# SketchyScene/SketchySceneColorization

Hardware: AMD Instinct MI355X
Metric: train images/sec (192x192, gen+disc fwd+bwd) (higher is better)
Workload: dtype fp32 (bf16x6 split on the bf16 MFMA, fp32 accumulate; filter gradients and few-channel layers on the exact-fp32 MFMA); 1 GPU; Foreground_Instance_Colorization Pix2Pix GAN train step (D-step + G-step, TF-Adam), 192x192, batch 32 per GPU; global_batch=32, parallelism=dp1, ranks_observed_by_allreduce=1, launcher=in-process, block_type=Pix2Pix, launch=hipGraph replay

## Files before the change

include/sketchycolor_hip.h:

```cpp
#ifndef SKETCHYCOLOR_HIP_H
#define SKETCHYCOLOR_HIP_H

#include <stdint.h>

#ifdef __cplusplus
extern "C" {
#endif

#define SSC_ACT_NONE 0
#define SSC_ACT_RELU 1
#define SSC_ACT_LRELU 2
#define SSC_ACT_TANH 3
#define SSC_ACT_PRELU 5
#define SSC_ACT_MIU 4

typedef struct ssc_gview {
    const float* s0;
    const float* s1;
    const float* ab0;
    const float* ab1;
    int32_t C0, C1;
    int32_t H, W;
    int32_t act;
    int32_t act1;
// ... 38 lines not shown
    int32_t ws_kc;
    const void* wsplit;
    int32_t ws_nbp;
    int32_t lds_hint;
} ssc_conv_desc;
#define SSC_SK_FLAG_WORDS 8192
typedef struct ssc_split_job {
    const float* w;
    void* dst;
    int32_t taps, c0, c1, orient;
    int64_t first_thread;
} ssc_split_job;
int ssc_filter_split_geom(int taps, int c0, int c1, int orient, int* kc, int* nbp, int64_t* bytes, int64_t* threads);
int ssc_filter_split(const float* w, int taps, int c0, int c1, int orient, void* dst, void* stream);
int ssc_bf16_prepare(void);
int ssc_filter_split_batch(const ssc_split_job* jobs_dev, int njobs, int64_t total_threads, void* stream);

int ssc_sk_configure(int timeout_ms, int test_withhold);

typedef struct ssc_wgrad_desc {
    ssc_gview g;
    ssc_gview d;
    float* out;
    int32_t NB, PH, PW;
    int32_t TH, TW, in_stride, ioff_y, ioff_x;
    int32_t Cg_real;
    int32_t Nn;
    int32_t ldc;
    int32_t accumulate;
    int32_t exact;
    int32_t _pad;
} ssc_wgrad_desc;

int ssc_version(void);
int ssc_build_hash(char* buf, int len);
int ssc_device_info(int* cu_count, int* wave_size, char* arch, int arch_len);

int ssc_conv_forward(const ssc_conv_desc* d, float* ws, int64_t ws_bytes, void* stream);
int ssc_conv_wgrad(const ssc_wgrad_desc* d, float* ws, int64_t ws_bytes, void* stream);
int ssc_conv_wgrad128_supported(const ssc_wgrad_desc* d);
int ssc_conv_wgrad128(const ssc_wgrad_desc* d, float* ws, int64_t ws_bytes, void* stream);
int ssc_conv_wgn16_supported(const ssc_wgrad_desc* d);
int ssc_conv_forward_bn(const ssc_conv_desc* d, float* ws, int64_t ws_bytes, const float* scale, const float* offset,
                        float eps, float* ab, float* stats, void* stream);
int ssc_head1_forward_supported(const ssc_conv_desc* d);
int ssc_head1_forward(const ssc_conv_desc* d, float* ws, int64_t ws_bytes, void* stream);
int ssc_head1_dgrad_supported(const ssc_conv_desc* d);
int ssc_head1_dgrad(const ssc_conv_desc* d, void* stream);
int ssc_head1_wgrad_supported(const ssc_wgrad_desc* d);
int ssc_head1_wgrad(const ssc_wgrad_desc* d, float* ws, int64_t ws_bytes, void* stream);
int ssc_head1_dgrad_bn_backward(const ssc_conv_desc* d, const float* x, const float* ab, const float* stats, int act,
                                const float* rowb, float rowb_scale, float* dx, float* dscale, float* doffset, float* ws,
                                int64_t ws_bytes, void* stream);
int ssc_bn_bwd_finalize(const float* partial, int nblk, int C, int64_t M, float* coef, float* dscale, float* doffset,
                        void* stream);
int ssc_conv_narrow_supported(const ssc_conv_desc* d);
int ssc_conv_narrow_forward(const ssc_conv_desc* d, void* stream);
int ssc_conv_pw1x1_supported(const ssc_conv_desc* d);
int ssc_conv_c3x3_supported(const ssc_conv_desc* d);
int ssc_conv_s2n16_supported(const ssc_conv_desc* d);
int ssc_conv_tr4n16_supported(const ssc_conv_desc* d);
int ssc_conv_fewchan7_supported(const ssc_conv_desc* d);
int ssc_conv_tr4_tiny_supported(const ssc_conv_desc* d);
int ssc_conv_fewchan_supported(const ssc_conv_desc* d);
int ssc_conv_forward_kernel_name(const ssc_conv_desc* d, char* buf, int len);
int ssc_conv_wgrad_kernel_name(const ssc_wgrad_desc* d, char* buf, int len);
int ssc_conv_forward_plan(const ssc_conv_desc* d, int64_t ws_bytes, int* out5);
#define SSC_RIDER_BN 0
#define SSC_RIDER_BNBWD 1
#define SSC_RIDER_BNBWD2 2
#define SSC_RIDER_MINMAX 3
#define SSC_RIDER_PATH_PLAIN 0
#define SSC_RIDER_PATH_STREAM 1
#define SSC_RIDER_PATH_TILE 2
#define SSC_RIDER_PATH_SLAB 3
#define SSC_RIDER_ROWS_NONE 0
#define SSC_RIDER_ROWS_WS_HEAD 1
#define SSC_RIDER_ROWS_WS_TAIL 2
#define SSC_RIDER_ROWS_CALLER 3
struct ssc_bnbwd_site;
int ssc_conv_rider_plan(const ssc_conv_desc* d, int rider, int64_t ws_bytes, const struct ssc_bnbwd_site* site0,
                        const struct ssc_bnbwd_site* site1, int C0, int64_t* out5);
int ssc_conv_wgrad_plan(const ssc_wgrad_desc* d, int64_t ws_bytes, int* out4);
int ssc_conv_wgrad128_plan(const ssc_wgrad_desc* d, int64_t ws_bytes, int* out7);
int ssc_conv_bf_plan(const ssc_conv_desc* d, int64_t ws_bytes, int* out10);
int ssc_conv_stream_plan(const ssc_conv_desc* d, int* out4);

int ssc_nchw_to_nhwc(const float* src, float* dst, int N, int C, int HW, int ldc, int coff, void* stream);
int ssc_nhwc_to_nchw(const float* src, float* dst, int N, int C, int HW, int ldc, int coff, void* stream);
int ssc_sketch_preprocess_u8(const uint8_t* src, int N, int H, int W, int thicken, float* dst, void* stream);
int ssc_image_postprocess_u8(const float* src, int ldc, int coff, int64_t M, uint8_t* dst, void* stream);
int ssc_bg_stage_u8(const uint8_t* fg, const uint8_t* bg, const int32_t* labels, int64_t M, float* inputs, float* targets,
                    float* xd_real, float* count, void* workspace, int64_t workspace_bytes, void* stream);
int ssc_bg_stage_cached_u8(const uint8_t* fg_cache, int64_t S_fg, const uint8_t* bg_cache, int64_t S_bg, const uint8_t* seg_cache,
                           int64_t S_seg, const int32_t* slot, const uint8_t* recolor, int64_t N, int64_t P, float* inputs,
                           float* targets, float* xd_real, int32_t* labels, float* count, void* workspace,
                           int64_t workspace_bytes, void* stream);
int ssc_bg_finish_u8(const float* img, int ldc, const uint8_t* fg, const uint8_t* mask, int64_t M, uint8_t* out,
                     void* stream);
int ssc_image_metrics_u8(const uint8_t* a, const uint8_t* b, const uint8_t* mask, int N, int H, int W, const double* win11,
                         double* out, void* ws, int64_t ws_bytes, void* stream);
int ssc_image_metrics_f32(const float* a, int lda, int coff_a, const float* b, int ldb, int coff_b, int b_planar, int N, int H,
                          int W, const double* win11, double* out, void* ws, int64_t ws_bytes, void* stream);
int ssc_image_metrics_bg_f32(const float* img, int ldc, const uint8_t* fg, const uint8_t* target, const uint8_t* mask, int N, int H,
                             int W, const double* win11, double* out, void* ws, int64_t ws_bytes, void* stream);
int ssc_color_metrics_u8(const uint8_t* a, const uint8_t* b, const uint8_t* mask, int N, int H, int W, const double* lin256,
// ... 244 lines not shown
```

sketchyscenecolorization_amd/build.py:

```python
import os
import subprocess
import sys

HERE = os.path.dirname(os.path.abspath(__file__))
ROOT = os.path.dirname(HERE)
CSRC = os.path.join(HERE, 'csrc')
LIB_DIR = os.path.join(HERE, 'lib')
LIB_PATH = os.path.join(LIB_DIR, 'libsketchycolor_hip.so')
EXTRA_FLAGS = {'igemm.hip': ['-Xclang', '-target-feature', '-Xclang', '-load-store-opt']} if os.environ.get('SSC_NO_LSOPT') == '1' else {}
NO_PACKED_FP32 = {'narrow.hip': []}
VGPR_FORM = ['-mllvm', '-amdgpu-mfma-vgpr-form=1']
LAST_BUILD = None
SOURCES = ['igemm.hip', 'igemm_bf16.hip', 'wgrad128.hip', 'wgrad128_bf16.hip', 'wgn16.hip', 'narrow.hip', 'head1.hip', 'fewchan.hip', 'fewchan7.hip', 'pw1x1.hip', 'c3x3.hip', 's2n16.hip', 'tr4tiny.hip', 'tr4n16.hip', 'elementwise.hip', 'text_lstm.hip', 'losses_optim.hip', 'mru_ops.hip', 'bg_io.hip', 'bg_scene.hip', 'fg_scene.hip', 'metrics.hip', 'color_metrics.hip', 'matching.hip', 'match_eval.hip', 'match_train.hip', 'match_val.hip', 'match_backbone_train.hip', 'match_attn.hip', 'match_segnet.hip', 'scene_system.hip', 'preview.hip']


def _hipcc():
    for c in (os.environ.get('HIPCC'), '/opt/rocm/bin/hipcc', 'hipcc'):
        if c and (os.path.isabs(c) and os.path.exists(c) or not os.path.isabs(c)):
            return c
    return 'hipcc'


HASH_MARKER = b'SSC_CSRC_HASH='


def tree_hash(csrc=None, header=None):
    import hashlib
    csrc = csrc or CSRC
    header = header or os.path.join(ROOT, 'include', 'sketchycolor_hip.h')
    h = hashlib.sha256()
    for fp in [os.path.join(csrc, f) for f in sorted(os.listdir(csrc))] + [header]:
        if fp.endswith(('.hip', '.h')):
            with open(fp, 'rb') as fh:
                h.update(os.path.basename(fp).encode() + b'\0' + fh.read())
    return h.hexdigest()[:16]


def library_hash(path=None):
    path = path or LIB_PATH
    if not os.path.exists(path):
        return None
    with open(path, 'rb') as fh:
        blob = fh.read()
    i = blob.find(HASH_MARKER)
    if i < 0:
        return None
    return blob[i + len(HASH_MARKER):i + len(HASH_MARKER) + 16].decode('ascii', 'replace')


def is_stale():
    return library_hash() != tree_hash()


def build_library(force=False, verbose=True):
    global LAST_BUILD
    if not force and not is_stale():
        LAST_BUILD = 'reused'
        return LIB_PATH
    LAST_BUILD = 'rebuilt'
    os.makedirs(LIB_DIR, exist_ok=True)
    th = tree_hash()
    import hashlib
    objs = []
    procs = []
    hdrs = b''
    for hp in sorted(os.path.join(CSRC, f) for f in os.listdir(CSRC) if f.endswith('.h')) + [os.path.join(ROOT, 'include', 'sketchycolor_hip.h')]:
# ... 36 lines not shown
```

sketchyscenecolorization_amd/hip.py:

```python
import ctypes as C
import os

import torch

_HERE = os.path.dirname(os.path.abspath(__file__))
LIB_PATH = os.environ.get('SSC_LIB_PATH') or os.path.join(_HERE, 'lib', 'libsketchycolor_hip.so')

ACT_PRELU = 5
ACT_NONE, ACT_RELU, ACT_LRELU, ACT_TANH, ACT_MIU = 0, 1, 2, 3, 4


class GView(C.Structure):
    _fields_ = [('s0', C.c_void_p), ('s1', C.c_void_p), ('ab0', C.c_void_p), ('ab1', C.c_void_p),
                ('C0', C.c_int32), ('C1', C.c_int32), ('H', C.c_int32), ('W', C.c_int32),
                ('act', C.c_int32), ('act1', C.c_int32)]


class ConvDesc(C.Structure):
    _fields_ = [('x', GView), ('w', C.c_void_p), ('bias', C.c_void_p), ('out', C.c_void_p),
                ('NB', C.c_int32), ('PH', C.c_int32), ('PW', C.c_int32),
                ('TH', C.c_int32), ('TW', C.c_int32), ('in_stride', C.c_int32),
                ('ioff_y', C.c_int32), ('ioff_x', C.c_int32), ('nphase', C.c_int32),
                ('ky0', C.c_int32), ('kx0', C.c_int32), ('kstep', C.c_int32),
                ('KH', C.c_int32), ('KW', C.c_int32), ('wC0', C.c_int32), ('wC1', C.c_int32),
                ('bmode', C.c_int32), ('k_real', C.c_int32), ('n_off', C.c_int32), ('Nn', C.c_int32),
                ('Nstore', C.c_int32), ('OH', C.c_int32), ('OW', C.c_int32), ('ldc', C.c_int32),
                ('out_stride', C.c_int32), ('ooff_y', C.c_int32), ('ooff_x', C.c_int32),
                ('epi', C.c_int32), ('accumulate', C.c_int32), ('stat_partial', C.c_void_p), ('sk_flags', C.c_void_p),
                ('sb_x', C.c_void_p), ('sb_ab', C.c_void_p), ('sb_stats', C.c_void_p), ('sb_ldx', C.c_int32),
                ('sb_act', C.c_int32), ('sk_tag', C.c_int32), ('sb2_col0', C.c_int32),
                ('sb2_x', C.c_void_p), ('sb2_ab', C.c_void_p), ('sb2_stats', C.c_void_p), ('stat_partial2', C.c_void_p),
                ('sb2_ldx', C.c_int32), ('sb2_act', C.c_int32),
                ('stat_mode', C.c_int32), ('ws_kc', C.c_int32),
                ('wsplit', C.c_void_p), ('ws_nbp', C.c_int32), ('lds_hint', C.c_int32)]


class SplitJob(C.Structure):
    _fields_ = [('w', C.c_void_p), ('dst', C.c_void_p), ('taps', C.c_int32), ('c0', C.c_int32), ('c1', C.c_int32),
                ('orient', C.c_int32), ('first_thread', C.c_int64)]


class BnApplyJob(C.Structure):
    _fields_ = [('x', C.c_void_p), ('M', C.c_int64), ('C', C.c_int32), ('ldx', C.c_int32), ('ab', C.c_void_p),
                ('stats', C.c_void_p), ('g1', C.c_void_p), ('g2', C.c_void_p), ('ldg1', C.c_int32), ('act1', C.c_int32),
                ('ldg2', C.c_int32), ('act2', C.c_int32), ('has_bn', C.c_int32), ('rowb_P', C.c_int32), ('rowb', C.c_void_p),
                ('rowb_scale', C.c_float), ('lddx', C.c_int32), ('coef', C.c_void_p), ('dx', C.c_void_p)]


class BnBwdSite(C.Structure):
    _fields_ = [('x', C.c_void_p), ('ab', C.c_void_p), ('stats', C.c_void_p), ('partial', C.c_void_p),
                ('partial_bytes', C.c_int64), ('ldx', C.c_int32), ('act', C.c_int32)]


class WgradDesc(C.Structure):
    _fields_ = [('g', GView), ('d', GView), ('out', C.c_void_p),
                ('NB', C.c_int32), ('PH', C.c_int32), ('PW', C.c_int32),
                ('TH', C.c_int32), ('TW', C.c_int32), ('in_stride', C.c_int32),
                ('ioff_y', C.c_int32), ('ioff_x', C.c_int32),
                ('Cg_real', C.c_int32), ('Nn', C.c_int32), ('ldc', C.c_int32), ('accumulate', C.c_int32),
                ('exact', C.c_int32), ('_pad', C.c_int32)]


_lib = None


def _dev_env(name, default=None):
    return os.environ.get(name, default) if os.environ.get('SSC_DEV_SWITCHES') == '1' else default


def lib():
    global _lib
    if _lib is None:
        if not os.path.exists(LIB_PATH):
            raise RuntimeError('libsketchycolor_hip.so is missing (%s): run `python -c "import __graft_entry__ as g; '
                               'g.build()"` or `python -m sketchyscenecolorization_amd.build`' % LIB_PATH)
        l = C.CDLL(LIB_PATH)
        _declare(l)
        check_build_hash(l)
        _lib = l
    return _lib


def build_hash(l=None):
    buf = C.create_string_buffer(32)
    (l if l is not None else lib()).ssc_build_hash(buf, 32)
    return buf.value.decode()


def check_build_hash(l=None, tree=None):
    from . import build
    have = build_hash(l)
    if tree is None:
        try:
            tree = build.tree_hash()
        except OSError:
            import warnings
            warnings.warn('%s: kernel sources not found beside the package, build hash %s not checked' % (LIB_PATH, have))
            return have
    want = tree
    if have != want:
        msg = ('%s was built from kernel sources %s, the tree is %s: rebuild (python -m sketchyscenecolorization_amd.build)'
               % (LIB_PATH, have, want))
        if os.environ.get('SSC_ALLOW_STALE_LIB') == '1':
            import warnings
            warnings.warn(msg)
        else:
            raise RuntimeError(msg)
    return have


_P, _I, _L, _F = C.c_void_p, C.c_int, C.c_int64, C.c_float

SIGNATURES = {
    'ssc_version': [],
    'ssc_build_hash': [C.c_char_p, _I],
    'ssc_device_info': [C.POINTER(C.c_int), C.POINTER(C.c_int), C.c_char_p, _I],
    'ssc_conv_forward': [C.POINTER(ConvDesc), _P, _L, _P],
    'ssc_filter_split_geom': [_I, _I, _I, _I, C.POINTER(C.c_int), C.POINTER(C.c_int), C.POINTER(C.c_int64), C.POINTER(C.c_int64)],
    'ssc_filter_split': [_P, _I, _I, _I, _I, _P, _P],
    'ssc_filter_split_batch': [_P, _I, _L, _P],
    'ssc_bf16_prepare': [],
    'ssc_conv_wgrad': [C.POINTER(WgradDesc), _P, _L, _P],
    'ssc_conv_wgrad128_supported': [C.POINTER(WgradDesc)],
    'ssc_conv_wgn16_supported': [C.POINTER(WgradDesc)],
    'ssc_conv_wgrad128': [C.POINTER(WgradDesc), _P, _L, _P],
    'ssc_conv_forward_bn': [C.POINTER(ConvDesc), _P, _L, _P, _P, _F, _P, _P, _P],
    'ssc_bn_finalize': [_P, _I, _I, _L, _P, _P, _F, _P, _P, _P],
    'ssc_conv_forward_bnbwd': [C.POINTER(ConvDesc), _P, _L, _P, _I, _P, _P, _I, _P, _L, C.POINTER(C.c_int), _P],
    'ssc_conv_forward_minmax': [C.POINTER(ConvDesc), _P, _L, _P, _P],
    'ssc_minmax_finalize': [_P, _I, _I, _I, _P, _P],
    'ssc_conv_forward_bnbwd2': [C.POINTER(ConvDesc), _P, _L, C.POINTER(BnBwdSite), C.POINTER(BnBwdSite), _I,
                                C.POINTER(C.c_int), _P],
    'ssc_bn_act_backward_pre': [_P, _L, _I, _I, _P, _P, _P, _I, _I, _P, _I, _I, _I, _P, _I, _P, _P, _P, _I, _P, _F, _I, _P,
                                _L, _P],
    'ssc_head1_forward_supported': [C.POINTER(ConvDesc)],
    'ssc_head1_forward': [C.POINTER(ConvDesc), _P, _L, _P],
    'ssc_head1_dgrad_supported': [C.POINTER(ConvDesc)],
    'ssc_head1_dgrad': [C.POINTER(ConvDesc), _P],
    'ssc_head1_wgrad_supported': [C.POINTER(WgradDesc)],
    'ssc_head1_wgrad': [C.POINTER(WgradDesc), _P, _L, _P],
    'ssc_head1_dgrad_bn_backward': [C.POINTER(ConvDesc), _P, _P, _P, _I, _P, _F, _P, _P, _P, _P, _L, _P],
    'ssc_bn_bwd_finalize': [_P, _I, _I, _L, _P, _P, _P, _P],
    'ssc_block_out_backward': [_P, _P, _L, _I, _I, _P, _P, _P, _P, _P, _P, _P, _P, _P, _P, _P, _P, _P, _P, _P, _L, _P],
    'ssc_bn_bwd_sums': [C.POINTER(BnApplyJob), _P, _I, _P, _P, _P, _P, _L, _P],
    'ssc_bn_bwd_apply': [C.POINTER(BnApplyJob), _P],
    'ssc_conv_narrow_supported': [C.POINTER(ConvDesc)],
    'ssc_conv_narrow_forward': [C.POINTER(ConvDesc), _P],
    'ssc_conv_fewchan_supported': [C.POINTER(ConvDesc)],
    'ssc_conv_pw1x1_supported': [C.POINTER(ConvDesc)],
    'ssc_conv_c3x3_supported': [C.POINTER(ConvDesc)],
    'ssc_conv_s2n16_supported': [C.POINTER(ConvDesc)],
    'ssc_conv_tr4n16_supported': [C.POINTER(ConvDesc)],
    'ssc_conv_fewchan7_supported': [C.POINTER(ConvDesc)],
    'ssc_conv_tr4_tiny_supported': [C.POINTER(ConvDesc)],
    'ssc_conv_forward_kernel_name': [C.POINTER(ConvDesc), C.c_char_p, _I],
    'ssc_conv_wgrad_kernel_name': [C.POINTER(WgradDesc), C.c_char_p, _I],
    'ssc_conv_forward_plan': [C.POINTER(ConvDesc), _L, C.POINTER(C.c_int)],
    'ssc_conv_rider_plan': [C.POINTER(ConvDesc), _I, _L, C.POINTER(BnBwdSite), C.POINTER(BnBwdSite), _I, C.POINTER(C.c_int64)],
    'ssc_conv_wgrad_plan': [C.POINTER(WgradDesc), _L, C.POINTER(C.c_int)],
    'ssc_conv_wgrad128_plan': [C.POINTER(WgradDesc), _L, C.POINTER(C.c_int)],
    'ssc_conv_bf_plan': [C.POINTER(ConvDesc), _L, C.POINTER(C.c_int)],
    'ssc_conv_stream_plan': [C.POINTER(ConvDesc), C.POINTER(C.c_int)],
    'ssc_sk_configure': [_I, _I],
    'ssc_nchw_to_nhwc': [_P, _P, _I, _I, _I, _I, _I, _P],
    'ssc_nhwc_to_nchw': [_P, _P, _I, _I, _I, _I, _I, _P],
    'ssc_sketch_preprocess_u8': [_P, _I, _I, _I, _I, _P, _P],
    'ssc_image_postprocess_u8': [_P, _I, _I, _L, _P, _P],
    'ssc_bg_stage_u8': [_P, _P, _P, _L, _P, _P, _P, _P, _P, _L, _P],
    'ssc_bg_stage_cached_u8': [_P, _L, _P, _L, _P, _L, _P, _P, _L, _L, _P, _P, _P, _P, _P, _P, _L, _P],
    'ssc_bg_finish_u8': [_P, _I, _P, _P, _L, _P, _P],
    'ssc_bg_scene_crop_u8': [_P, _P, _L, _P, _P],
    'ssc_bg_scene_compose_u8': [_P, _I, _P, _P, _P, _P, _I, _I, _P, _P, _I, _P],
    'ssc_bg_sky_gradient_u8': [_P, _P, _I, _I, _I, _I, _P, _P, _P, _L, _P],
    'ssc_fg_scene_mask_u8': [_P, _I, _I, _P, _P],
    'ssc_road_parallel_u8': [_P, _I, _I, _P, _P],
    'ssc_fg_scene_paste_u8': [_P, _P, _I, _I, _P, _I, _I, _I, _I, _I, _P],
    'ssc_image_metrics_u8': [_P, _P, _P, _I, _I, _I, _P, _P, _P, _L, _P],
    'ssc_image_metrics_f32': [_P, _I, _I, _P, _I, _I, _I, _I, _I, _I, _P, _P, _P, _L, _P],
    'ssc_image_metrics_bg_f32': [_P, _I, _P, _P, _P, _I, _I, _I, _P, _P, _P, _L, _P],
    'ssc_color_metrics_u8': [_P, _P, _P, _I, _I, _I, _P, _P, _P, _P, _L, _P],
    'ssc_color_metrics_f32': [_P, _I, _I, _P, _I, _I, _I, _I, _I, _I, _P, _P, _P, _P, _L, _P],
    'ssc_color_metrics_bg_f32': [_P, _I, _P, _P, _P, _I, _I, _I, _P, _P, _P, _P, _L, _P],
    'ssc_seg_confusion': [_P, _I, _I, _P, _L, _L, _P, _P, _L, _P],
    'ssc_resample_u8': [_P, _I, _I, _I, _I, _P, _P, _I, _I, _P, _P, _I, _I, _P, _P, _I, _I, _I, _I, _I, _I, _P],
    'ssc_decode_paired_u8': [_P, _P, _P, _I, _I, _I, _P, _P, _P, _P, _P],
    'ssc_decode_minmax_u8': [_P, _I, _I, _I, _P, _P],
    'ssc_decode_paired_cached_u8': [_P, _P, _P, _P, _L, _P, _I, _I, _I, _P, _P, _P, _P],
    'ssc_distance_map_u8': [_P, _I, _I, _P, _P, _L, _P],
    'ssc_fill': [_P, _F, _L, _P],
    'ssc_timestamp': [_P, _P],
    'ssc_affine_act': [_P, _I, _P, _I, _I, _P, _I, _L, _I, _P],
    'ssc_residual_merge': [_P, _P, _P, _P, _I, _P, _L, _I, _P],
    'ssc_bn_stats': [_P, _L, _I, _I, _P, _P, _F, _P, _P, _P, _L, _P],
    'ssc_bn_act_backward': [_P, _L, _I, _I, _P, _P, _P, _P, _I, _I, _P, _I, _I, _I, _P, _I, _P, _P, _P, _L, _P],
# ... 689 lines not shown
    if not lib().ssc_head1_dgrad_supported(C.byref(d)):
        return False
    ws = workspace()
    check(lib().ssc_head1_dgrad_bn_backward(C.byref(d), ptr(x4d), ptr(ab), ptr(stats), act,
                                            ptr(rowb[0]) if rowb else None, float(rowb[1]) if rowb else 0.0, ptr(dx4d),
                                            ptr(dscale), ptr(doffset), ptr(ws), ws.numel() * 4, stream_ptr()),
          'ssc_head1_dgrad_bn_backward')
    return True


def deconv_dgrad(dy, f, out, n_off=0, nn=None, accumulate=False, bnbwd=None):
    KH, KW, co, ci = f.shape
    nn = ci - n_off if nn is None else nn
    d = ConvDesc()
    d.x = dy.c()
    d.w, d.bias = f.data_ptr(), None
    d.out, OH, OW, ldc = _out_geom(out, 0)
    d.NB, d.PH, d.PW = dy.N, dy.H // 2, dy.W // 2
    assert (OH, OW) == (d.PH, d.PW) and co <= dy.C
    d.TH, d.TW, d.in_stride, d.ioff_y, d.ioff_x, d.nphase = 4, 4, 2, -1, -1, 1
    d.ky0, d.kx0, d.kstep = 0, 0, 1
    d.KH, d.KW, d.wC0, d.wC1, d.bmode, d.k_real = 4, 4, co, ci, 0, co
    d.n_off, d.Nn, d.Nstore = n_off, nn, nn
    d.OH, d.OW, d.ldc, d.out_stride, d.ooff_y, d.ooff_x = OH, OW, ldc, 1, 0, 0
    d.epi, d.accumulate = 0, int(accumulate)
    _attach_split(d, f)
    _run_conv(d, bnbwd=bnbwd)


def conv_wgrad(x, dy, w_grad, stride, pad, accumulate=False):
    KH, KW, ci, co = w_grad.shape
    d = WgradDesc()
    d.g, d.d = x.c(), dy.c()
    d.out = w_grad.data_ptr()
    d.NB, d.PH, d.PW = dy.N, dy.H, dy.W
    d.TH, d.TW, d.in_stride, d.ioff_y, d.ioff_x = KH, KW, stride, -pad, -pad
    d.Cg_real, d.Nn, d.ldc, d.accumulate = ci, co, co, int(accumulate)
    assert ci <= x.C and co <= dy.C
    _run_wgrad(d, side=True)


def deconv_wgrad(x, dy, f_grad, accumulate=False):
    KH, KW, co, ci = f_grad.shape
    d = WgradDesc()
    d.g, d.d = dy.c(), x.c()
    d.out = f_grad.data_ptr()
    d.NB, d.PH, d.PW = x.N, x.H, x.W
    d.TH, d.TW, d.in_stride, d.ioff_y, d.ioff_x = 4, 4, 2, -1, -1
    d.Cg_real, d.Nn, d.ldc, d.accumulate = co, ci, ci, int(accumulate)
    assert co <= dy.C and ci <= x.C
    _run_wgrad(d, side=True)


def _mat_view(a, ab=None, act=ACT_NONE):
    assert a.dim() == 2 and a.is_contiguous()
    return View(a.view(1, 1, a.shape[0], a.shape[1]), None, ab, act)


def matmul(a, b, out, bias=None, accumulate=False, a_ab=None, a_act=ACT_NONE):
    M, K = a.shape
    K2, N = b.shape
    assert K == K2 and out.shape == (M, N) and out.is_contiguous()
    conv_forward(_mat_view(a, a_ab, a_act), b.view(1, 1, K, N), 1, 0, out.view(1, 1, M, N), bias=bias,
                 accumulate=accumulate)


def matmul_nt(a, b, out, accumulate=False):
    M, K = a.shape
    N, K2 = b.shape
    assert K == K2 and out.shape == (M, N)
    d = ConvDesc()
    d.x = _mat_view(a).c()
    d.w, d.bias, d.out = b.data_ptr(), None, out.data_ptr()
    d.NB, d.PH, d.PW, d.TH, d.TW, d.in_stride, d.ioff_y, d.ioff_x, d.nphase = 1, 1, M, 1, 1, 1, 0, 0, 1
    d.ky0, d.kx0, d.kstep, d.KH, d.KW, d.wC0, d.wC1, d.bmode, d.k_real = 0, 0, 1, 1, 1, N, K, 1, K
    d.n_off, d.Nn, d.Nstore, d.OH, d.OW, d.ldc, d.out_stride, d.ooff_y, d.ooff_x = 0, N, N, 1, M, N, 1, 0, 0
    d.epi, d.accumulate = 0, int(accumulate)
    _attach_split(d, b.view(1, 1, N, K))
    _run_conv(d)


def matmul_tn(a, b, out, accumulate=False, a_ab=None, a_act=ACT_NONE):
    M, K = a.shape
    M2, N = b.shape
    assert M == M2 and out.shape == (K, N) and out.is_contiguous()
    d = WgradDesc()
    d.g, d.d = _mat_view(a, a_ab, a_act).c(), _mat_view(b).c()
    d.out = out.data_ptr()
    d.NB, d.PH, d.PW, d.TH, d.TW, d.in_stride, d.ioff_y, d.ioff_x = 1, 1, M, 1, 1, 1, 0, 0
    d.Cg_real, d.Nn, d.ldc, d.accumulate = K, N, N, int(accumulate)
    _run_wgrad(d)


def nchw_to_nhwc(src, dst, coff=0):
    n, c, h, w = src.shape
    assert dst.shape[:3] == (n, h, w) and src.is_contiguous() and dst.is_contiguous()
    check(lib().ssc_nchw_to_nhwc(ptr(src), ptr(dst), n, c, h * w, dst.shape[3], coff, stream_ptr()), 'nchw_to_nhwc')


def nhwc_to_nchw(src, dst, coff=0):
    n, c, h, w = dst.shape
    assert src.shape[:3] == (n, h, w) and src.is_contiguous() and dst.is_contiguous()
    check(lib().ssc_nhwc_to_nchw(ptr(src), ptr(dst), n, c, h * w, src.shape[3], coff, stream_ptr()), 'nhwc_to_nchw')


def sketch_preprocess_u8(src_u8, thicken=False, out=None):
# ... 937 lines not shown
```

sketchyscenecolorization_amd/pix2pix.py:

```python
import torch

from . import hip
from .hip import _dev_env
from .hip import ACT_LRELU, ACT_NONE, ACT_RELU, View
from .net_common import SnClassHead, _rows
from .text_fusion import TextFusion


class Pix2PixGenerator(object):

    def __init__(self, store, bufs, lstm_hybrid=True):
        self.s, self.b = store, bufs
        self.lstm_hybrid = bool(lstm_hybrid)
        self.text_stream = None
        self.text_stream_bwd = None
        self.text = TextFusion(store, bufs)

    def forward(self, sketches, text, noise_vec, tag='g', out=None, out_coff=0):
        s, B = self.s, self.b
        nhwc_in = sketches.dim() == 4 and sketches.shape[3] == 4 and sketches.shape[1] != 3
        N, H, W = (sketches.shape[0], sketches.shape[1], sketches.shape[2]) if nhwc_in else \
            (sketches.shape[0], sketches.shape[2], sketches.shape[3])
        chans = [None, 64, 128, 256, 512, 512]
        tstream = self.text_stream if hip.PROFILE is None else None
# ... 131 lines not shown
        dpre_fc = B.get(tag + '/gb/noise_dpre', (N, cd * P))
        hip.call('ssc_miu_permute_bwd', ctx['noise_pre'], g_noise, N, cd, P, dpre_fc)
        hip.matmul_tn(ctx['noise_vec'], dpre_fc, s.grad('generator/fully_connected/weights'))
        hip.call('ssc_group_rowsum', dpre_fc, cd * P, 1, N, cd * P, s.grad('generator/fully_connected/biases'), 0)
        hip.mark(tag + '/bwd decoders dgrad: last')
        if held:
            main = torch.cuda.current_stream()
            side_stream.wait_stream(main)
            with torch.cuda.stream(side_stream):
                for wg in held:
                    wg()
        else:
            done('decoders')
        de5 = B.get(tag + '/gb/de5', e[5].shape)
        text_pending = False
        if self.lstm_hybrid:
            tstream = self.text_stream_bwd if hip.PROFILE is None else None
            dy5 = self.text.backward(ctx['tctx'], g_feat, side_stream=tstream)
            hip.mark(tag + '/bwd caption branch: last (main stream)')
            if held:
                main.wait_stream(side_stream)
                hip.mark(tag + '/bwd held decoder wgrads joined')
                done('decoders')
            if tstream is None:
                done('text')
            else:
                text_pending = True
            if dy5 is None:
                hip.fill(de5, 0.0)
                hip.fill(s.grad('generator/encoder_5/scale'), 0.0)
                hip.fill(s.grad('generator/encoder_5/offset'), 0.0)
            else:
                hip.bn_act_backward(_rows(e[5]), ab[5], st[5], dy5, ACT_NONE, _rows(de5),
                                    dscale=s.grad('generator/encoder_5/scale'),
                                    doffset=s.grad('generator/encoder_5/offset'))
        else:
            for nm in ('embedding', 'RNN/WLSTM/multi_rnn_cell/cell_0/basic_lstm_cell/kernel',
                       'RNN/WLSTM/multi_rnn_cell/cell_0/basic_lstm_cell/bias',
                       'RNN/ALSTM/multi_rnn_cell/cell_0/basic_lstm_cell/kernel',
                       'RNN/ALSTM/multi_rnn_cell/cell_0/basic_lstm_cell/bias'):
                hip.fill(s.grad('generator/TextLSTM/' + nm), 0.0)
            done('text')
            hip.bn_act_backward(_rows(e[5]), ab[5], st[5], _rows(g_feat), ACT_RELU, _rows(de5),
                                dscale=s.grad('generator/encoder_5/scale'),
                                doffset=s.grad('generator/encoder_5/offset'))
        gcur = de5
        for k in (5, 4, 3, 2):
            w = s['generator/encoder_%d/conv/filter' % k]
            xin = View(e[k - 1], None, ab[k - 1], ACT_LRELU)
            dyv = View(gcur)
            gin = B.get(tag + '/gb/e%d_in' % k, e[k - 1].shape)
            live = sums_e[k - 1] is not None and not sums_e[k - 1].missed
            hip.conv_dgrad(dyv, w, 2, 1, gin, bnbwd=(sums_e[k - 1].take(ACT_LRELU) if live else None))
            dx = B.get(tag + '/gb/de%d' % (k - 1), e[k - 1].shape)
            hip.conv_wgrad(xin, dyv, s.grad('generator/encoder_%d/conv/filter' % k), 2, 1)
            if k - 1 >= 2:
                hip.bn_act_backward(_rows(e[k - 1]), ab[k - 1], st[k - 1], _rows(gin), ACT_LRELU, _rows(dx),
                                    g2=_rows(g_skip[k - 1]), act2=ACT_RELU,
                                    dscale=s.grad('generator/encoder_%d/scale' % (k - 1)),
                                    doffset=s.grad('generator/encoder_%d/offset' % (k - 1)), pre=sums_e[k - 1])
            else:
                hip.bn_act_backward(_rows(e[1]), None, None, _rows(gin), ACT_LRELU, _rows(dx),
                                    g2=_rows(g_skip[1]), act2=ACT_RELU)
            gcur = dx
            if k == 5 and not text_pending:
                done('encoder_5')
        hip.conv_wgrad(View(ctx['xs']), View(gcur), s.grad('generator/encoder_1/conv/filter'), 2, 1)
        hip.mark(tag + '/bwd encoders: last')
        if text_pending:
            self.text.join_backward()
            done('text')
            done('encoder_5')
        done('encoders')


_HEAD1_FUSED = _dev_env('SSC_HEAD1_FUSED', '0') == '1'


class Pix2PixDiscriminator(SnClassHead):

    def __init__(self, store, bufs, sn=True):
        self.s, self.b = store, bufs
        self.sn = bool(sn)
        self.chans = [8, 64, 128, 256, 512, 1]
        self.strides = [None, 2, 2, 2, 1, 1]

    def forward(self, xd, sn, tag):
        s, B = self.s, self.b
        N, H, W, _ = xd.shape
        l, ab, st = [None] * 6, [None] * 6, [None] * 6
        l[0] = xd
        h, w = H, W
        for k in range(1, 6):
            if self.strides[k] == 2:
                h, w = h // 2, w // 2
            else:
                h, w = h - 1, w - 1
            co = self.chans[k]
            l[k] = B.get(tag + '/l%d' % k, (N, h, w, 4 if k == 5 else co))
            if k == 1:
                v = View(xd)
            elif k == 2:
                v = View(l[1], None, None, ACT_LRELU)
            else:
                v = View(l[k - 1], None, ab[k - 1], ACT_LRELU)
            bn = None
            if 2 <= k <= 4:
                ab[k] = B.get(tag + '/ab%d' % k, (2 * co,))
                st[k] = B.get(tag + '/st%d' % k, (2 * co,))
                bn = (s['discriminator/layer_%d/scale' % k], s['discriminator/layer_%d/offset' % k], ab[k], st[k])
            hip.conv_forward(v, s['discriminator/layer_%d/conv/filter' % k], self.strides[k], 1, l[k],
                             nstore=(4 if k == 5 else None), bn=bn)
        P4 = l[4].shape[1] * l[4].shape[2]
        img = B.get(tag + '/img', (N, 512))
        hip.call('ssc_act_mean_hw', l[4], ab[4], ACT_LRELU, N, P4, 512, img)
        logits = self._head_forward(tag, img, sn)
        return {'tag': tag, 'N': N, 'l': l, 'ab': ab, 'st': st, 'img': img, 'logits': logits, 'disc': l[5], 'P4': P4}

    def backward(self, ctx, dl5, dlogits, sn, need_params, need_input, accumulate, after_layer=None, stop_after=None,
                 resume=None):
        s, B = self.s, self.b
        tag, N, l, ab, st = ctx['tag'], ctx['N'], ctx['l'], ctx['ab'], ctx['st']
        gname = lambda k, what: s.grad('discriminator/layer_%d/%s' % (k, what))
        if resume is not None:
            return self._backward_layers(ctx, resume['layers'], resume['gcur'], resume['sums'], None, None, need_params,
                                         need_input, accumulate, after_layer, None)
        x5 = View(l[4], None, ab[4], ACT_LRELU)
        dy5 = View(dl5)
        if need_params:
            hip.conv_wgrad(x5, dy5, gname(5, 'conv/filter'), 1, 1, accumulate=accumulate)
        rowb = None
        if dlogits is not None:
            dimg = self._head_backward(ctx, sn, dlogits, need_params, accumulate)
            rowb = (dimg, 1.0 / ctx['P4'], ctx['P4'])
        return self._backward_layers(ctx, (4, 3, 2, 1), None, None, dy5, rowb, need_params, need_input, accumulate, after_layer,
                                     stop_after)

    def _norm_backward(self, ctx, k, gcur, sums, need_params, accumulate, rowb=None):
        s, B = self.s, self.b
        tag, l, ab, st = ctx['tag'], ctx['l'], ctx['ab'], ctx['st']
        gname = lambda kk, what: s.grad('discriminator/layer_%d/%s' % (kk, what))
        dx = B.get(tag + '/gb/dl%d' % k, l[k].shape)
        if k == 1:
            hip.bn_act_backward(_rows(l[1]), None, None, _rows(gcur), ACT_LRELU, _rows(dx))
            return dx
        ds = do = None
        if need_params and accumulate:
            tmp_s = B.get(tag + '/gb/tmp_scale%d' % k, (2, self.chans[k]))
            ds, do = tmp_s[0], tmp_s[1]
        elif need_params:
            ds, do = gname(k, 'scale'), gname(k, 'offset')
        hip.bn_act_backward(_rows(l[k]), ab[k], st[k], _rows(gcur), ACT_LRELU, _rows(dx), dscale=ds, doffset=do, pre=sums,
                            rowb=rowb)
        if need_params and accumulate:
            hip.call('ssc_axpy', gname(k, 'scale'), ds, 1.0, self.chans[k])
            hip.call('ssc_axpy', gname(k, 'offset'), do, 1.0, self.chans[k])
        return dx

    def _backward_layers(self, ctx, layers, dx, sums, dy5, rowb, need_params, need_input, accumulate, after_layer, stop_after):
        s, B = self.s, self.b
        tag, N, l, ab, st = ctx['tag'], ctx['N'], ctx['l'], ctx['ab'], ctx['st']
        gname = lambda k, what: s.grad('discriminator/layer_%d/%s' % (k, what))
        dgen = None
        if dx is None:
            assert layers[0] == 4
            dx = B.get(tag + '/gb/dl4', l[4].shape)
            ds = do = None
            if need_params and accumulate:
                tmp_s = B.get(tag + '/gb/tmp_scale4', (2, self.chans[4]))
                ds, do = tmp_s[0], tmp_s[1]
            elif need_params:
                ds, do = gname(4, 'scale'), gname(4, 'offset')
            fused = _HEAD1_FUSED and hip.head1_dgrad_bn_backward(dy5, s['discriminator/layer_5/conv/filter'], 1, l[4], ab[4], st[4],
                                                                 ACT_LRELU, dx, dscale=ds, doffset=do,
                                                                 rowb=(rowb[:2] if rowb else None))
            if not fused:
                g4 = B.get(tag + '/gb/g4', l[4].shape)
                hip.conv_dgrad(dy5, s['discriminator/layer_5/conv/filter'], 1, 1, g4, k_real=1)
                hip.bn_act_backward(_rows(l[4]), ab[4], st[4], _rows(g4), ACT_LRELU, _rows(dx), dscale=ds, doffset=do, rowb=rowb)
            if need_params and accumulate:
                hip.call('ssc_axpy', gname(4, 'scale'), ds, 1.0, self.chans[4])
                hip.call('ssc_axpy', gname(4, 'offset'), do, 1.0, self.chans[4])
        for k in layers:
            if k == 1:
                xin = View(l[0])
            elif k == 2:
                xin = View(l[1], None, None, ACT_LRELU)
            else:
                xin = View(l[k - 1], None, ab[k - 1], ACT_LRELU)
            dyv = View(dx)
            w = s['discriminator/layer_%d/conv/filter' % k]
            dx_next = None
            if need_params:
                hip.conv_wgrad(xin, dyv, gname(k, 'conv/filter'), self.strides[k], 1, accumulate=accumulate)
                if after_layer is not None:
                    after_layer(k)
            if k > 1:
                gin = B.get(tag + '/gb/g%d' % (k - 1), l[k - 1].shape)
                sums = None
                if k - 1 >= 2:
                    x2d = _rows(l[k - 1])
                    sums = hip.BnBwdSums(x2d, ab[k - 1], st[k - 1],
                                         B.get(tag + '/gb/bnsums%d' % (k - 1),
                                               (hip.BnBwdSums.rows_needed(x2d.shape[0]), 2 * x2d.shape[1])))
                hip.conv_dgrad(dyv, w, self.strides[k], 1, gin, bnbwd=(sums.take(ACT_LRELU) if sums else None))
                dx_next = self._norm_backward(ctx, k - 1, gin, sums, need_params, accumulate)
            elif need_input:
                dgen = B.get(tag + '/gb/dgen', (N, l[0].shape[1], l[0].shape[2], 4))
                hip.conv_dgrad(dyv, w, 2, 1, dgen, n_off=3, nn=3, nstore=4)
            dx = dx_next
            if stop_after == k and k > 1:
                return {'layers': tuple(j for j in layers if j < k), 'gcur': dx, 'sums': None}
        return dgen
```

Before: 2376 images/sec.

## Fuse first-layer activation backward into a dedicated first-layer wgrad kernel

Adds a specialized weight-gradient kernel for the first 4x4 stride-2 conv (4 or 8 input channels, 64 outputs). It applies the LReLU/ReLU derivative of the layer output on the fly, summing two gradient streams where needed, and feeds the result into fp32 MFMA with LDS-staged input patches and a cross-block slab reduction. The generator encoder_1 and discriminator layer_1 paths now skip materializing the activation-backward tensor and the separate generic wgrad launch, which saves a full-resolution write and read. The cost is an extra reduction kernel, workspace use, and new fallback branches in Python.

Result: no change. 2392 images/sec (median of 6 runs) (+0.7%).

```diff
diff --git a/include/sketchycolor_hip.h b/include/sketchycolor_hip.h
--- a/include/sketchycolor_hip.h
+++ b/include/sketchycolor_hip.h
@@ -114,6 +114,20 @@
 int ssc_head1_dgrad_bn_backward(const ssc_conv_desc* d, const float* x, const float* ab, const float* stats, int act,
                                 const float* rowb, float rowb_scale, float* dx, float* dscale, float* doffset, float* ws,
                                 int64_t ws_bytes, void* stream);
+typedef struct ssc_first_wgrad_desc {
+    const float* x;
+    const float* y;
+    const float* g1;
+    const float* g2;
+    float* out;
+    int32_t NB, PH, PW;
+    int32_t Cs;
+    int32_t ci_real;
+    int32_t act1, act2;
+    int32_t accumulate;
+} ssc_first_wgrad_desc;
+int ssc_first_layer_wgrad_supported(const ssc_first_wgrad_desc* d);
+int ssc_first_layer_wgrad(const ssc_first_wgrad_desc* d, void* ws, int64_t ws_bytes, void* stream);
 int ssc_bn_bwd_finalize(const float* partial, int nblk, int C, int64_t M, float* coef, float* dscale, float* doffset,
                         void* stream);
 int ssc_conv_narrow_supported(const ssc_conv_desc* d);
diff --git a/sketchyscenecolorization_amd/build.py b/sketchyscenecolorization_amd/build.py
--- a/sketchyscenecolorization_amd/build.py
+++ b/sketchyscenecolorization_amd/build.py
@@ -11,7 +11,7 @@
 NO_PACKED_FP32 = {'narrow.hip': []}
 VGPR_FORM = ['-mllvm', '-amdgpu-mfma-vgpr-form=1']
 LAST_BUILD = None
-SOURCES = ['igemm.hip', 'igemm_bf16.hip', 'wgrad128.hip', 'wgrad128_bf16.hip', 'wgn16.hip', 'narrow.hip', 'head1.hip', 'fewchan.hip', 'fewchan7.hip', 'pw1x1.hip', 'c3x3.hip', 's2n16.hip', 'tr4tiny.hip', 'tr4n16.hip', 'elementwise.hip', 'text_lstm.hip', 'losses_optim.hip', 'mru_ops.hip', 'bg_io.hip', 'bg_scene.hip', 'fg_scene.hip', 'metrics.hip', 'color_metrics.hip', 'matching.hip', 'match_eval.hip', 'match_train.hip', 'match_val.hip', 'match_backbone_train.hip', 'match_attn.hip', 'match_segnet.hip', 'scene_system.hip', 'preview.hip']
+SOURCES = ['igemm.hip', 'igemm_bf16.hip', 'wgrad128.hip', 'wgrad128_bf16.hip', 'wgn16.hip', 'wgrad_first.hip', 'narrow.hip', 'head1.hip', 'fewchan.hip', 'fewchan7.hip', 'pw1x1.hip', 'c3x3.hip', 's2n16.hip', 'tr4tiny.hip', 'tr4n16.hip', 'elementwise.hip', 'text_lstm.hip', 'losses_optim.hip', 'mru_ops.hip', 'bg_io.hip', 'bg_scene.hip', 'fg_scene.hip', 'metrics.hip', 'color_metrics.hip', 'matching.hip', 'match_eval.hip', 'match_train.hip', 'match_val.hip', 'match_backbone_train.hip', 'match_attn.hip', 'match_segnet.hip', 'scene_system.hip', 'preview.hip']
 
 
 def _hipcc():
diff --git a/sketchyscenecolorization_amd/csrc/wgrad_first.hip b/sketchyscenecolorization_amd/csrc/wgrad_first.hip
--- /dev/null
+++ b/sketchyscenecolorization_amd/csrc/wgrad_first.hip
@@ -0,0 +1,271 @@
+#include <hip/hip_runtime.h>
+#include "sketchycolor_hip.h"
+#include "bn_bwd.h"
+
+#define CHECK_LAUNCH() ((int)hipGetLastError())
+
+typedef float fw_v4f __attribute__((ext_vector_type(4)));
+
+constexpr int FW_THREADS = 512;
+constexpr int FW_WAVES = FW_THREADS / 64;
+constexpr int FW_MAX_SLABS = 256;
+constexpr int FW_BUF_F4 = 2560;
+constexpr int FW_NU = FW_BUF_F4 / FW_THREADS;
+constexpr int FW_RING = 3;
+
+struct FwPlan {
+    int RC;
+    int cpi;
+    int nch;
+    int cps;
+    int slabs;
+    int G4;
+    int ipc;
+    int Wl;
+    int rowf4;
+};
+
+struct FwArgs {
+    const float* x; const float* y; const float* g1; const float* g2;
+    float* partial;
+    int NB, PH, PW;
+    float s1, s2;
+    FwPlan p;
+};
+
+static bool fw_plan(const ssc_first_wgrad_desc* d, FwPlan* p) {
+    if (d == nullptr || d->x == nullptr || d->y == nullptr || d->g1 == nullptr || d->out == nullptr) return false;
+    if (d->Cs != 4 && d->Cs != 8) return false;
+    if (d->ci_real < 1 || d->ci_real > d->Cs || d->NB < 1 || d->PH < 1 || d->PW < 1) return false;
+    if ((long)d->NB * d->PH * d->PW * 64 >= (1L << 31)) return false;
+    const int pwp = (d->PW + 3) & ~3;
+    p->G4 = pwp / 4;
+    p->Wl = 2 * pwp + 2;
+    p->rowf4 = p->Wl * d->Cs / 4;
+    p->RC = 0;
+    for (int rc = 4; rc >= 1; rc >>= 1)
+        if ((2 * rc + 2) * p->rowf4 <= FW_BUF_F4) { p->RC = rc; break; }
+    if (p->RC == 0) return false;
+    if (p->RC > d->PH) p->RC = d->PH >= 2 ? 2 : 1;
+    p->cpi = (d->PH + p->RC - 1) / p->RC;
+    p->nch = d->NB * p->cpi;
+    const int s0 = p->nch < FW_MAX_SLABS ? p->nch : FW_MAX_SLABS;
+    p->cps = (p->nch + s0 - 1) / s0;
+    p->slabs = (p->nch + p->cps - 1) / p->cps;
+    const int ipc = (p->RC * p->G4 + FW_WAVES - 1) / FW_WAVES;
+    p->ipc = (ipc + FW_RING - 1) / FW_RING * FW_RING;
+    return true;
+}
+
+struct FwChunk { int n, py0, rc; };
+
+__device__ __forceinline__ FwChunk fw_chunk(const FwArgs& a, int cid, int c_end) {
+    FwChunk c;
+    c.n = 0; c.py0 = 0; c.rc = 0;
+    if (cid < c_end) {
+        c.n = cid / a.p.cpi;
+        c.py0 = (cid - c.n * a.p.cpi) * a.p.RC;
+        c.rc = min(a.p.RC, a.PH - c.py0);
+    }
+    return c;
+}
+
+template <bool TWO>
+struct FwItem { float4 y, g1, g2; };
+
+template <bool TWO>
+__device__ __forceinline__ void fw_load(const FwArgs& a, const FwChunk& c, int g, int k, int j, FwItem<TWO>& it) {
+    const bool group_ok = g < c.rc * a.p.G4;
+    const int gg = group_ok ? g : 0;
+    const int pyl = gg / a.p.G4;
+    const int px = (gg - pyl * a.p.G4) * 4 + k;
+    long off = (((long)c.n * a.PH + c.py0 + pyl) * a.PW + px) * 64 + 4 * j;
+    if (!group_ok || px >= a.PW) off = 4 * j;
+    it.y = *reinterpret_cast<const float4*>(a.y + off);
+    it.g1 = *reinterpret_cast<const float4*>(a.g1 + off);
+    if (TWO) it.g2 = *reinterpret_cast<const float4*>(a.g2 + off);
+}
+
+__device__ __forceinline__ float fw_dz(float y, float g1, float g2, bool two, float s1, float s2) {
+    float t = 0.f;
+    if (two) t = fmaf(g2, y > 0.f ? 1.f : s2, t);
+    return fmaf(g1, y > 0.f ? 1.f : s1, t);
+}
+
+template <int CS, bool TWO>
+__global__ __launch_bounds__(FW_THREADS) void first_wgrad_kernel(FwArgs a) {
+    constexpr int MT = CS;
+    __shared__ float4 lds4[2 * FW_BUF_F4];
+    const float* ldsf = reinterpret_cast<const float*>(lds4);
+    const int tid = threadIdx.x, lane = tid & 63;
+    const int wave = __builtin_amdgcn_readfirstlane(tid >> 6);
+    const int k = lane >> 4, j = lane & 15;
+    const FwPlan& p = a.p;
+    const int c_begin = blockIdx.x * p.cps;
+    const int c_end = min(c_begin + p.cps, p.nch);
+    const int H = 2 * a.PH, W = 2 * a.PW;
+
+    const int a_lane = j + 2 * k * CS;
+    int a_tile[MT];
+#pragma unroll
+    for (int mt = 0; mt < MT; ++mt) a_tile[mt] = (CS == 4 ? mt : mt >> 1) * p.Wl * CS + (CS == 8 ? 16 * (mt & 1) : 0);
+
+    fw_v4f acc[MT][4];
+#pragma unroll
+    for (int mt = 0; mt < MT; ++mt)
+#pragma unroll
+        for (int r = 0; r < 4; ++r) acc[mt][r] = fw_v4f{0.f, 0.f, 0.f, 0.f};
+
+    float4 xr[FW_NU];
+    unsigned xmask = 0;
+    auto xload = [&](const FwChunk& c) {
+        const int nunits = (2 * c.rc + 2) * p.rowf4;
+        xmask = 0;
+#pragma unroll
+        for (int u = 0; u < FW_NU; ++u) {
+            const int idx = tid + u * FW_THREADS;
+            const int row = idx / p.rowf4, rem = idx - row * p.rowf4;
+            const int col = rem / (CS / 4), q = rem - col * (CS / 4);
+            const int iy = 2 * c.py0 - 1 + row, ix = col - 1;
+            const bool ok = idx < nunits && iy >= 0 && iy < H && ix >= 0 && ix < W;
+            const long off = ok ? (((long)c.n * H + iy) * W + ix) * CS + 4 * q : 0;
+            xr[u] = *reinterpret_cast<const float4*>(a.x + off);
+            xmask |= ok ? 1u << u : 0u;
+        }
+    };
+    auto xstore = [&](const FwChunk& c, int buf) {
+        const int nunits = (2 * c.rc + 2) * p.rowf4;
+#pragma unroll
+        for (int u = 0; u < FW_NU; ++u) {
+            const int idx = tid + u * FW_THREADS;
+            const bool ok = (xmask >> u) & 1u;
+            const float4 v = make_float4(ok ? xr[u].x : 0.f, ok ? xr[u].y : 0.f, ok ? xr[u].z : 0.f, ok ? xr[u].w : 0.f);
+            if (idx < nunits) lds4[buf * FW_BUF_F4 + idx] = v;
+        }
+    };
+
+    FwChunk cur = fw_chunk(a, c_begin, c_end);
+    FwChunk nxt = fw_chunk(a, c_begin + 1, c_end);
+    FwItem<TWO> ring[FW_RING];
+#pragma unroll
+    for (int d = 0; d < FW_RING; ++d) fw_load<TWO>(a, cur, wave + FW_WAVES * d, k, j, ring[d]);
+    xload(cur);
+
+    for (int cid = c_begin; cid < c_end; ++cid) {
+        const int buf = (cid - c_begin) & 1;
+        xstore(cur, buf);
+        __syncthreads();
+        xload(nxt);
+        const float* patch = ldsf + buf * (FW_BUF_F4 * 4) + a_lane;
+        for (int t0 = 0; t0 < p.ipc; t0 += FW_RING) {
+#pragma unroll
+            for (int d = 0; d < FW_RING; ++d) {
+                const int t = t0 + d;
+                const int g = wave + FW_WAVES * t;
+                if (g < cur.rc * p.G4) {
+                    const int pyl = g / p.G4, gx = g - pyl * p.G4;
+                    const float* pa = patch + (2 * pyl * p.Wl + 8 * gx) * CS;
+                    float av[MT];
+#pragma unroll
+                    for (int mt = 0; mt < MT; ++mt) av[mt] = pa[a_tile[mt]];
+                    const FwItem<TWO>& it = ring[d];
+                    const bool in_row = 4 * gx + k < a.PW;
+                    float dz[4];
+                    dz[0] = in_row ? fw_dz(it.y.x, it.g1.x, TWO ? it.g2.x : 0.f, TWO, a.s1, a.s2) : 0.f;
+                    dz[1] = in_row ? fw_dz(it.y.y, it.g1.y, TWO ? it.g2.y : 0.f, TWO, a.s1, a.s2) : 0.f;
+                    dz[2] = in_row ? fw_dz(it.y.z, it.g1.z, TWO ? it.g2.z : 0.f, TWO, a.s1, a.s2) : 0.f;
+                    dz[3] = in_row ? fw_dz(it.y.w, it.g1.w, TWO ? it.g2.w : 0.f, TWO, a.s1, a.s2) : 0.f;
+#pragma unroll
+                    for (int mt = 0; mt < MT; ++mt)
+#pragma unroll
+                        for (int r = 0; r < 4; ++r)
+                            acc[mt][r] = __builtin_amdgcn_mfma_f32_16x16x4f32(av[mt], dz[r], acc[mt][r], 0, 0, 0);
+                }
+                if (t + FW_RING < p.ipc) fw_load<TWO>(a, cur, g + FW_WAVES * FW_RING, k, j, ring[d]);
+                else fw_load<TWO>(a, nxt, wave + FW_WAVES * (t + FW_RING - p.ipc), k, j, ring[d]);
+            }
+        }
+        cur = nxt;
+        nxt = fw_chunk(a, cid + 2, c_end);
+    }
+
+    float4* red = lds4;
+    float4* slab = reinterpret_cast<float4*>(a.partial) + (long)blockIdx.x * (16 * CS * 16);
+    __syncthreads();
+    for (int wv = 0; wv < FW_WAVES; ++wv) {
+        if (wave == wv) {
+#pragma unroll
+            for (int mt = 0; mt < MT; ++mt)
+#pragma unroll
+                for (int rr = 0; rr < 4; ++rr) {
+                    const int idx = (16 * mt + 4 * k + rr) * 16 + j;
+                    float4 v = make_float4(acc[mt][0][rr], acc[mt][1][rr], acc[mt][2][rr], acc[mt][3][rr]);
+                    if (wv > 0) {
+                        const float4 o = red[idx];
+                        v.x = o.x + v.x; v.y = o.y + v.y; v.z = o.z + v.z; v.w = o.w + v.w;
+                    }
+                    if (wv < FW_WAVES - 1) red[idx] = v;
+                    else slab[idx] = v;
+                }
+        }
+        __syncthreads();
+    }
+}
+
+__global__ __launch_bounds__(256) void first_wgrad_reduce_kernel(const float* __restrict__ partial, int slabs, int Cs, int ci_real,
+                                                                  float* __restrict__ out, int accumulate) {
+    __shared__ float sh[4][64];
+    const int co = threadIdx.x & 63, q = threadIdx.x >> 6;
+    const int m = blockIdx.x;
+    const long per_slab = 16L * Cs * 64;
+    const float* src = partial + (long)m * 64 + co;
+    float s = 0.f;
+#pragma unroll 8
+    for (int sl = q; sl < slabs; sl += 4) s += src[sl * per_slab];
+    sh[q][co] = s;
+    __syncthreads();
+    const int tap = m / Cs, ci = m - tap * Cs;
+    if (q == 0 && ci < ci_real) {
+        const float tot = ((sh[0][co] + sh[1][co]) + sh[2][co]) + sh[3][co];
+        float* o = out + ((long)tap * ci_real + ci) * 64 + co;
+        *o = accumulate ? *o + tot : tot;
+    }
+}
+
+static float fw_slope(int act) { return act == SSC_ACT_RELU ? 0.f : (act == SSC_ACT_LRELU ? 0.2f : 1.f); }
+
+extern "C" int ssc_first_layer_wgrad_supported(const ssc_first_wgrad_desc* d) {
+    FwPlan p;
+    if (!fw_plan(d, &p)) return 0;
+    const int acts_ok = (d->act1 == SSC_ACT_NONE || d->act1 == SSC_ACT_RELU || d->act1 == SSC_ACT_LRELU) &&
+                        (d->g2 == nullptr || d->act2 == SSC_ACT_NONE || d->act2 == SSC_ACT_RELU || d->act2 == SSC_ACT_LRELU);
+    return acts_ok ? 1 : 0;
+}
+
+extern "C" int ssc_first_layer_wgrad(const ssc_first_wgrad_desc* d, void* ws, int64_t ws_bytes, void* stream) {
+    FwPlan p;
+    if (!ssc_first_layer_wgrad_supported(d) || !fw_plan(d, &p)) return -1;
+    const int64_t need = (int64_t)p.slabs * 16 * d->Cs * 64 * (int64_t)sizeof(float);
+    if (ws == nullptr || ws_bytes < need) return -2;
+    FwArgs a;
+    a.x = d->x; a.y = d->y; a.g1 = d->g1; a.g2 = d->g2;
+    a.partial = static_cast<float*>(ws);
+    a.NB = d->NB; a.PH = d->PH; a.PW = d->PW;
+    a.s1 = fw_slope(d->act1); a.s2 = fw_slope(d->act2);
+    a.p = p;
+    hipStream_t st = (hipStream_t)stream;
+    const dim3 grid((unsigned)p.slabs), block(FW_THREADS);
+    const bool two = d->g2 != nullptr;
+    if (d->Cs == 4) {
+        if (two) hipLaunchKernelGGL((first_wgrad_kernel<4, true>), grid, block, 0, st, a);
+        else hipLaunchKernelGGL((first_wgrad_kernel<4, false>), grid, block, 0, st, a);
+    } else {
+        if (two) hipLaunchKernelGGL((first_wgrad_kernel<8, true>), grid, block, 0, st, a);
+        else hipLaunchKernelGGL((first_wgrad_kernel<8, false>), grid, block, 0, st, a);
+    }
+    int rc = CHECK_LAUNCH();
+    if (rc != 0) return rc;
+    hipLaunchKernelGGL(first_wgrad_reduce_kernel, dim3(16 * d->Cs), dim3(256), 0, st, a.partial, p.slabs, d->Cs, d->ci_real,
+                       d->out, d->accumulate);
+    return CHECK_LAUNCH();
+}
diff --git a/sketchyscenecolorization_amd/hip.py b/sketchyscenecolorization_amd/hip.py
--- a/sketchyscenecolorization_amd/hip.py
+++ b/sketchyscenecolorization_amd/hip.py
@@ -59,6 +59,12 @@
                 ('ioff_y', C.c_int32), ('ioff_x', C.c_int32),
                 ('Cg_real', C.c_int32), ('Nn', C.c_int32), ('ldc', C.c_int32), ('accumulate', C.c_int32),
                 ('exact', C.c_int32), ('_pad', C.c_int32)]
+
+
+class FirstWgradDesc(C.Structure):
+    _fields_ = [('x', C.c_void_p), ('y', C.c_void_p), ('g1', C.c_void_p), ('g2', C.c_void_p), ('out', C.c_void_p),
+                ('NB', C.c_int32), ('PH', C.c_int32), ('PW', C.c_int32), ('Cs', C.c_int32), ('ci_real', C.c_int32),
+                ('act1', C.c_int32), ('act2', C.c_int32), ('accumulate', C.c_int32)]
 
 
 _lib = None
@@ -140,6 +146,8 @@
     'ssc_head1_wgrad_supported': [C.POINTER(WgradDesc)],
     'ssc_head1_wgrad': [C.POINTER(WgradDesc), _P, _L, _P],
     'ssc_head1_dgrad_bn_backward': [C.POINTER(ConvDesc), _P, _P, _P, _I, _P, _F, _P, _P, _P, _P, _L, _P],
+    'ssc_first_layer_wgrad_supported': [C.POINTER(FirstWgradDesc)],
+    'ssc_first_layer_wgrad': [C.POINTER(FirstWgradDesc), _P, _L, _P],
     'ssc_bn_bwd_finalize': [_P, _I, _I, _L, _P, _P, _P, _P],
     'ssc_block_out_backward': [_P, _P, _L, _I, _I, _P, _P, _P, _P, _P, _P, _P, _P, _P, _P, _P, _P, _P, _P, _P, _L, _P],
     'ssc_bn_bwd_sums': [C.POINTER(BnApplyJob), _P, _I, _P, _P, _P, _P, _L, _P],
@@ -935,6 +943,49 @@
     _run_wgrad(d, side=True)
 
 
+def first_layer_wgrad(x, y, g1, act1, w_grad, g2=None, act2=ACT_NONE, accumulate=False):
+    global _wgrad_pending
+    if w_grad.dim() != 4 or tuple(w_grad.shape[:2]) != (4, 4) or w_grad.shape[3] != 64 or not w_grad.is_contiguous():
+        return False
+    if x.s1 is not None or x.ab0 is not None or x.act != ACT_NONE:
+        return False
+    if y.dim() != 4 or y.shape[3] != 64 or (x.N, x.H, x.W) != (y.shape[0], 2 * y.shape[1], 2 * y.shape[2]):
+        return False
+    for t in (y, g1, g2):
+        if t is not None and not (t.is_contiguous() and t.shape == y.shape and t.dtype == torch.float32):
+            return False
+    d = FirstWgradDesc()
+    d.x, d.y, d.g1, d.g2, d.out = x.s0.data_ptr(), y.data_ptr(), g1.data_ptr(), (g2.data_ptr() if g2 is not None else None), \
+        w_grad.data_ptr()
+    d.NB, d.PH, d.PW, d.Cs, d.ci_real = y.shape[0], y.shape[1], y.shape[2], x.C0, w_grad.shape[2]
+    d.act1, d.act2, d.accumulate = act1, act2, int(accumulate)
+    if not lib().ssc_first_layer_wgrad_supported(C.byref(d)):
+        return False
+
+    def launch():
+        ws = workspace()
+        check(lib().ssc_first_layer_wgrad(C.byref(d), ptr(ws), ws.numel() * 4, stream_ptr()), 'ssc_first_layer_wgrad')
+
+    if WGRAD_STREAM is not None and PROFILE is None:
+        WGRAD_STREAM.wait_stream(torch.cuda.current_stream())
+        with torch.cuda.stream(WGRAD_STREAM):
+            launch()
+        _wgrad_pending = True
+        return True
+    if PROFILE is None:
+        launch()
+        return True
+    e0, e1 = torch.cuda.Event(enable_timing=True), torch.cuda.Event(enable_timing=True)
+    e0.record()
+    launch()
+    e1.record()
+    K = d.NB * d.PH * d.PW
+    flops = 2.0 * K * 16 * d.ci_real * 64
+    nbytes = 4.0 * (4 * K * d.Cs + K * 64 * (3 if g2 is not None else 2) + 16 * d.ci_real * 64 * (2 if accumulate else 1))
+    PROFILE.append(('first_layer_wgrad<%dx64>' % (16 * d.Cs), flops, e0, e1, (16 * d.ci_real, 64, K), nbytes))
+    return True
+
+
 def _mat_view(a, ab=None, act=ACT_NONE):
     assert a.dim() == 2 and a.is_contiguous()
     return View(a.view(1, 1, a.shape[0], a.shape[1]), None, ab, act)
diff --git a/sketchyscenecolorization_amd/pix2pix.py b/sketchyscenecolorization_amd/pix2pix.py
--- a/sketchyscenecolorization_amd/pix2pix.py
+++ b/sketchyscenecolorization_amd/pix2pix.py
@@ -207,20 +207,22 @@
             gin = B.get(tag + '/gb/e%d_in' % k, e[k - 1].shape)
             live = sums_e[k - 1] is not None and not sums_e[k - 1].missed
             hip.conv_dgrad(dyv, w, 2, 1, gin, bnbwd=(sums_e[k - 1].take(ACT_LRELU) if live else None))
-            dx = B.get(tag + '/gb/de%d' % (k - 1), e[k - 1].shape)
             hip.conv_wgrad(xin, dyv, s.grad('generator/encoder_%d/conv/filter' % k), 2, 1)
             if k - 1 >= 2:
+                dx = B.get(tag + '/gb/de%d' % (k - 1), e[k - 1].shape)
                 hip.bn_act_backward(_rows(e[k - 1]), ab[k - 1], st[k - 1], _rows(gin), ACT_LRELU, _rows(dx),
                                     g2=_rows(g_skip[k - 1]), act2=ACT_RELU,
                                     dscale=s.grad('generator/encoder_%d/scale' % (k - 1)),
                                     doffset=s.grad('generator/encoder_%d/offset' % (k - 1)), pre=sums_e[k - 1])
-            else:
+                gcur = dx
+            elif not hip.first_layer_wgrad(View(ctx['xs']), e[1], gin, ACT_LRELU, s.grad('generator/encoder_1/conv/filter'),
+                                           g2=g_skip[1], act2=ACT_RELU):
+                dx = B.get(tag + '/gb/de1', e[1].shape)
                 hip.bn_act_backward(_rows(e[1]), None, None, _rows(gin), ACT_LRELU, _rows(dx),
                                     g2=_rows(g_skip[1]), act2=ACT_RELU)
-            gcur = dx
+                hip.conv_wgrad(View(ctx['xs']), View(dx), s.grad('generator/encoder_1/conv/filter'), 2, 1)
             if k == 5 and not text_pending:
                 done('encoder_5')
-        hip.conv_wgrad(View(ctx['xs']), View(gcur), s.grad('generator/encoder_1/conv/filter'), 2, 1)
         hip.mark(tag + '/bwd encoders: last')
         if text_pending:
             self.text.join_backward()
@@ -279,7 +281,7 @@
         gname = lambda k, what: s.grad('discriminator/layer_%d/%s' % (k, what))
         if resume is not None:
             return self._backward_layers(ctx, resume['layers'], resume['gcur'], resume['sums'], None, None, need_params,
-                                         need_input, accumulate, after_layer, None)
+                                         need_input, accumulate, after_layer, None, raw1=resume.get('raw1', False))
         x5 = View(l[4], None, ab[4], ACT_LRELU)
         dy5 = View(dl5)
         if need_params:
@@ -312,7 +314,8 @@
             hip.call('ssc_axpy', gname(k, 'offset'), do, 1.0, self.chans[k])
         return dx
 
-    def _backward_layers(self, ctx, layers, dx, sums, dy5, rowb, need_params, need_input, accumulate, after_layer, stop_after):
+    def _backward_layers(self, ctx, layers, dx, sums, dy5, rowb, need_params, need_input, accumulate, after_layer, stop_after,
+                         raw1=False):
         s, B = self.s, self.b
         tag, N, l, ab, st = ctx['tag'], ctx['N'], ctx['l'], ctx['ab'], ctx['st']
         gname = lambda k, what: s.grad('discriminator/layer_%d/%s' % (k, what))
@@ -346,7 +349,13 @@
             dyv = View(dx)
             w = s['discriminator/layer_%d/conv/filter' % k]
             dx_next = None
-            if need_params:
+            if k == 1 and raw1:
+                if not hip.first_layer_wgrad(xin, l[1], dx, ACT_LRELU, gname(1, 'conv/filter'), accumulate=accumulate):
+                    hip.conv_wgrad(xin, View(self._norm_backward(ctx, 1, dx, None, need_params, accumulate)),
+                                   gname(1, 'conv/filter'), 2, 1, accumulate=accumulate)
+                if after_layer is not None:
+                    after_layer(1)
+            elif need_params:
                 hip.conv_wgrad(xin, dyv, gname(k, 'conv/filter'), self.strides[k], 1, accumulate=accumulate)
                 if after_layer is not None:
                     after_layer(k)
@@ -359,11 +368,12 @@
                                          B.get(tag + '/gb/bnsums%d' % (k - 1),
                                                (hip.BnBwdSums.rows_needed(x2d.shape[0]), 2 * x2d.shape[1])))
                 hip.conv_dgrad(dyv, w, self.strides[k], 1, gin, bnbwd=(sums.take(ACT_LRELU) if sums else None))
-                dx_next = self._norm_backward(ctx, k - 1, gin, sums, need_params, accumulate)
+                raw1 = k == 2 and need_params and not need_input
+                dx_next = gin if raw1 else self._norm_backward(ctx, k - 1, gin, sums, need_params, accumulate)
             elif need_input:
                 dgen = B.get(tag + '/gb/dgen', (N, l[0].shape[1], l[0].shape[2], 4))
                 hip.conv_dgrad(dyv, w, 2, 1, dgen, n_off=3, nn=3, nstore=4)
             dx = dx_next
             if stop_after == k and k > 1:
-                return {'layers': tuple(j for j in layers if j < k), 'gcur': dx, 'sums': None}
+                return {'layers': tuple(j for j in layers if j < k), 'gcur': dx, 'sums': None, 'raw1': raw1}
         return dgen
```
